# NERSC/swin_v2_weather

Hardware: AMD Instinct MI355X
Metric: ERA5 samples/sec (73x721x1440) swin_73var depth12 (higher is better)
Workload: dtype bf16

## Files before the change

### include/swv2.h

```cpp
#ifndef SWV2_H
#define SWV2_H
#include <stddef.h>
#include <stdint.h>

#ifdef __cplusplus
extern "C" {
#endif

#define SWV2_VERSION 113

enum {
    SWV2_OK = 0,
    SWV2_ERR_INVALID = -1,
    SWV2_ERR_UNSUPPORTED = -2,
    SWV2_ERR_LAUNCH = -3
};

int swv2_version(void);
const char* swv2_last_error(void);

int swv2_attn_geometry(int L, int head_dim, int* Lp, int* DP);

int swv2_attn_fwd_regime(int L, int head_dim, int has_bias, int dbg);

// ... 352 lines not shown
    const float* b2;
    const float* gamma;
    const float* beta;
    const float* scale;
    void* hpre;
    void* a2;
    float* mean;
    float* rstd;
    float* y;
    int M, C, hidden, rows_per_sample;
    float eps;
} swv2_mlp_args;
int swv2_mlp_supported(int C, int hidden);
int swv2_mlp_recompute_supported(int C, int hidden);
int swv2_mlp_fwd(const swv2_mlp_args* a, void* stream);

typedef struct {
    const float* dy;
    const void* a2;
    const float* mean;
    const float* rstd;
    const float* gamma;
    const float* scale;
    const void* hpre;
    const void* w2t;
    const void* w1t;
    void* da2;
    void* dh;
    float* dx;
    float* dgamma;
// ... 116 lines not shown
```

### swin_v2_weather_amd/_lib.py

```python
from __future__ import annotations

import ctypes as C
import os
import subprocess
import threading

HERE = os.path.dirname(os.path.abspath(__file__))
CSRC = os.path.join(HERE, "csrc")
LIB_PATH = os.environ.get("SWV2_LIB") or os.path.join(HERE, "libswv2.so")
SOURCES = ["capi.hip", "attn.hip", "attn2.hip", "attn_bwd_stream.hip", "attn_wide.hip", "attn_d256.hip", "gemm.hip", "gemm_rw.hip", "gemm_tn.hip", "gemm_tn_slab.hip", "rowops.hip", "lamb.hip", "block.hip", "cpb.hip", "mlp.hip", "proj_ln.hip", "dataio.hip", "packed.hip", "score.hip", "stats.hip", "quantile.hip", "ensemble.hip", "loss_l1.hip", "loss_l2.hip", "sht.hip", "regrid.hip", "events.hip", "fss.hip"]

ABI_VERSION = 113

_lib = None
_lock = threading.Lock()


class Swv2Error(RuntimeError):
    pass


def build_library(force: bool = False, verbose: bool = False) -> str:
    import glob
    srcs = [os.path.join(CSRC, s) for s in SOURCES]
# ... 257 lines not shown
    "swv2_era5_select_normalize": (_I, [_P, _P, _P, _P, _P] + [_I] * 10 + [_P]),
    "swv2_era5_zenith": (_I, [_P, _P, _I, _I, _I, _I, _I, _I, _P]),
    "swv2_era5_static": (_I, [_P, _P, _I, _I, _I, _I, _I, _I, _P]),
    "swv2_era5_select_normalize_i16": (_I, [_P] * 8 + [_I] * 10 + [_P]),
    "swv2_era5_unpack_i16": (_I, [_P, _P, _P, _P, _I, _I, _I, _P]),
    "swv2_era5_pack_i16": (_I, [_P, _P, _P, _P, _I, _I, _I, _P]),
    "swv2_pack_range_ws_bytes": (C.c_size_t, [_I, _I, _I]),
    "swv2_pack_range": (_I, [_P, _I, _I, _I, _I, _P, _P, _P, C.c_size_t, _P]),
    "swv2_proj_ln_supported": (_I, [_I, _I, _I]),
    "swv2_proj_ln_bwd_ws_floats": (C.c_size_t, [_I, _I]),
    "swv2_proj_ln_fwd": (_I, [C.POINTER(ProjLnArgs), _P]),
    "swv2_proj_ln_bwd": (_I, [C.POINTER(ProjLnBwdArgs), _P]),
    "swv2_mlp_supported": (_I, [_I, _I]),
    "swv2_mlp_recompute_supported": (_I, [_I, _I]),
    "swv2_mlp_fwd": (_I, [C.POINTER(MlpArgs), _P]),
    "swv2_mlp_bwd_ws_floats": (C.c_size_t, [_I, _I]),
    "swv2_mlp_bwd": (_I, [C.POINTER(MlpBwdArgs), _P]),
    "swv2_cpb_fwd": (_I, [_P, _P, _P, _P, _P, _P, _I, _I, _I, _I, _F, _P]),
    "swv2_cpb_bwd": (_I, [_P, _P, _P, _P, _P, _P, _P, _P, _P, _I, _I, _I, _I, _F, _P]),
    "swv2_cpb_bwd_ws": (_I, [_P, _P, _P, _P, _P, _P, _P, _P, _P, _I, _I, _I, _I, _F, _P, C.c_size_t, _P]),
    "swv2_cpb_bwd_ws_bytes": (C.c_size_t, [_I, _I, _I, _I]),
    "swv2_cpb_fwd_multi": (_I, [_P, _I, _P, _P, _I, _I, _I, _I, _F, _P]),
    "swv2_cpb_bwd_multi_ws_bytes": (C.c_size_t, [_I, _I, _I, _I, _I]),
    "swv2_cpb_bwd_multi": (_I, [_P, _I, _P, _I, _P, _P, _I, _I, _I, _I, _F, _P, C.c_size_t, _P]),
    "swv2_block_plan": (_I, [C.POINTER(BlockDesc), C.POINTER(BlockPlan)]),
    "swv2_block_step_id": (_I, [_I]),
    "swv2_block_step_name": (C.c_char_p, [_I]),
    "swv2_block_fwd": (_I, [C.POINTER(BlockDesc), _P]),
    "swv2_block_bwd": (_I, [C.POINTER(BlockDesc), _P]),
}
# ... 29 lines not shown
```

### swin_v2_weather_amd/csrc/gemm_common.h

```cpp
#pragma once
#include <cstdlib>
#include "common.h"

int swv2_tn_wide_launch(const swv2_operand* y, const swv2_operand* x, float* part, float* dbpart, int M, int N, int K, int S, hipStream_t st);

int swv2_rw_dx128_launch(const swv2_operand* a, const void* w, const swv2_epilogue* e, int M, hipStream_t st);

size_t swv2_tn_slab_ws_bytes(int C, int hidden, int heads_dp);
bool swv2_tn_slab_covers(const swv2_wgrad_item* it, size_t ws_bytes);
int swv2_tn_slab_launch(const swv2_wgrad_item* it, void* ws, size_t ws_bytes, const swv2_ln_partials* ln, hipStream_t st);

inline int swv2_env_switch(const char* name) { const char* v = getenv(name); return v ? atoi(v) : 1; }
inline int swv2_gemm_wide() { return swv2_env_switch("SWV2_GEMM_WIDE"); }
inline int swv2_wide_persist() { return swv2_env_switch("SWV2_WIDE_PERSIST"); }

namespace {

constexpr int BM = 128, BN = 128, BK = 64;
constexpr int KCH = BK / 8;
constexpr int NTHREADS = 256;

__device__ __forceinline__ int swz(int r, int kc) { return r * BK + ((kc ^ ((r >> 1) & 7)) << 3); }

__device__ __forceinline__ void erf_parts(float x, float& erf_v, float& gauss) {
    const float z = fabsf(x) * 0.70710678118654752f;
// ... 28 lines not shown
__device__ __forceinline__ uint16_t gelu_tab_arg(int i) { return (uint16_t)(((i / GT_HALF) << 15) | (GT_LO + i % GT_HALF)); }

template <int ESZ, bool SIGNED = true>
__device__ __forceinline__ uint32_t gelu_tab_off2(uint32_t w, bool& bad) {
    const u16x2_t a = __builtin_bit_cast(u16x2_t, w & 0x7fff7fffu);
    const u16x2_t lo = {(unsigned short)GT_LO, (unsigned short)GT_LO};
    const u16x2_t mx = {(unsigned short)(GT_HALF - 1), (unsigned short)(GT_HALF - 1)};
    const u16x2_t idx = a - lo;
    const u16x2_t idc = __builtin_elementwise_min(idx, mx);
    bad = bad || (__builtin_bit_cast(uint32_t, idx) != __builtin_bit_cast(uint32_t, idc));
    if constexpr (!SIGNED) return __builtin_bit_cast(uint32_t, (u16x2_t)(idc * (unsigned short)ESZ));
    const u16x2_t sg = __builtin_bit_cast(u16x2_t, w) >> 15;
    const u16x2_t half = {(unsigned short)GT_HALF, (unsigned short)GT_HALF};
    const u16x2_t off = (idc + sg * half) * (unsigned short)ESZ;
    return __builtin_bit_cast(uint32_t, off);
}

struct LoadDesc {
    const void* ptr;
    const int32_t* rowidx;
    const float* aux0;
    const float* aux1;
    const float* aux2;
    const float* aux3;
    long ld;
    int M, K;
    int p0, p1, p2, p3;
    uint32_t mg0, mg1, mg2;
};

// ... 258 lines not shown
```

### swin_v2_weather_amd/csrc/gemm_tn_slab.hip

```cpp
#include "gemm_common.h"
#pragma clang diagnostic ignored "-Wc++20-extensions"

namespace {

#ifdef SWV2_SLAB_PART_F32
typedef float sl_part_t;
#else
typedef uint16_t sl_part_t;
#endif
constexpr int SL_TH = 512;
constexpr int SL_SMEM = 160 * 1024;
constexpr int SL_IDX_CAP = 4096;
enum { F_ROW = 0, F_ROWG = 1, F_F32 = 2, F_F32G = 3, F_HEAD = 4 };

#ifdef SWV2_SLAB_STAMPS
#define SWV2_STAMPS
#endif
#include "stamps.h"

__device__ __forceinline__ uint4 sl_gelu8_tab(uint4 w, const unsigned char* tab0, bool& bad) {
    const uint32_t in[4] = {w.x, w.y, w.z, w.w};
    uint32_t out[4], off[4];
    u16x2_t mx = {0, 0};
    const u16x2_t lo = {(unsigned short)GT_LO, (unsigned short)GT_LO};
// ... 15 lines not shown

struct SlOp {
    const void* ptr;
    const int32_t* rowidx;
    int ld;
    int heads, parts, Lp, DP;
    uint32_t mgLp, mgDP, mgH;
};
struct SlProd {
    SlOp y, x;
    sl_part_t* part;
    float* dbpart;
    int M, N, K;
    int first, wgs, ntile;
};
struct SlArgs { SlProd p[4]; unsigned long long* stamps; };

template <int W>
__device__ __forceinline__ int sl_swz(int r, int u) {
    if constexpr ((W * 2) % 256 == 0) return u ^ (r & 7);
    else { static_assert((W * 2) % 128 == 0, "slab width"); return u ^ ((r >> 1) & 3); }
}

template <int FY, int FX, int TN, int TK, int WGN, int WGK, int SR, int NS, bool INPLACE = false>
__device__ __forceinline__ void slab_job(const SlProd& P, const int j, unsigned char* __restrict__ smem, [[maybe_unused]] unsigned long long* stamps) {
    static_assert(WGN * WGK == 8, "8 waves");
    constexpr int IA = TN / (16 * WGN), JB = TK / (16 * WGK);
    static_assert(IA * 16 * WGN == TN && JB * 16 * WGK == TK, "wave tiles");
    constexpr bool XF32 = FX == F_F32 || FX == F_F32G;
    constexpr int YP = TN * 2, XP = TK * 2;
    constexpr int YB = SR * TN * 2, XB = SR * TK * (XF32 ? 4 : 2), STG = YB + XB;
    constexpr int NY = YB / 1024, NX = XB / 1024, NTOT = NY + NX;
    static_assert(YB % 1024 == 0 && XB % 1024 == 0, "whole DMA instructions");
    constexpr int NIW = (NTOT + 7) / 8, NREM = NTOT % 8, D = NS - 1;
    constexpr int OFF_TAB = 0, TABB = FX == F_ROWG ? (GT_N * 2 + 1023) / 1024 * 1024 : 0;
    constexpr int OFF_IDX = OFF_TAB + TABB, IDXB = FX == F_F32G ? SL_IDX_CAP * 4 : 0;
    constexpr int OFF_SLOT = OFF_IDX + IDXB;
    constexpr int OFF_XB = OFF_SLOT + NS * STG, XBB = (XF32 && !INPLACE) ? SR * TK * 2 : 0;
    static_assert(OFF_XB + XBB <= SL_SMEM, "LDS budget");
    static_assert(!INPLACE || XF32, "in-place conversion: fp32 operands only");
    constexpr int KS = SR / 32;

    const int tid = threadIdx.x, lane = tid & 63, wave = __builtin_amdgcn_readfirstlane(tid >> 6);
    const int fr = lane & 15, g = lane >> 4;
    const int wgn = wave / WGK, wgk = wave - wgn * WGK;
    const int n_w = wgn * (TN / WGN), k_w = wgk * (TK / WGK);
    const int ntile = P.ntile, ntk = P.K / TK;
    const int slice = j / ntile, tile = j - slice * ntile, S = P.wgs / ntile;
    const int n0 = (tile / ntk) * TN, k0 = (tile % ntk) * TK;
    const int M = P.M, T = (M + SR - 1) / SR;
    const int nst = slice < T ? (T - slice + S - 1) / S : 0;
    auto stage_of = [&](int i) { return slice + i * S; };
    const uint32_t lds0 = (uint32_t)(uintptr_t)smem + OFF_SLOT;
    uint16_t* const xbs = (uint16_t*)(smem + OFF_XB);
    uint16_t* const tab = (uint16_t*)(smem + OFF_TAB);
    int32_t* const idxs = (int32_t*)(smem + OFF_IDX);

    if constexpr (FX == F_ROWG) {
        for (int i = tid; i < GT_N; i += SL_TH) tab[i] = f2bf(gelu_f(bf2f(gelu_tab_arg(i))));
    }
    constexpr int HS = SL_IDX_CAP / 2 / SR, RING = 2 * HS;
    auto fill_idx = [&](int h0) {
        for (int i = tid; i < HS * SR; i += SL_TH) {
            const int ti = h0 + i / SR;
            const int m = stage_of(ti) * SR + (i % SR);
            idxs[(ti % RING) * SR + (i % SR)] = (ti < nst && m < M) ? P.x.rowidx[m] : -1;
        }
    };
    if constexpr (FX == F_F32G) { fill_idx(0); fill_idx(HS); }
    if constexpr (FX == F_ROWG || FX == F_F32G) __syncthreads();

    int orow[NIW];
    uint32_t ocol[NIW];
#pragma unroll
    for (int q = 0; q < NIW; ++q) {
        const int ii = 8 * q + wave;
        if (ii < NY) {
            const int o = ii * 1024 + lane * 16;
            if constexpr (FY == F_ROW) {
                const int row = o / YP, rem = o - row * YP, pu = rem >> 5, u = sl_swz<TN>(row, pu);
                orow[q] = row; ocol[q] = (uint32_t)(n0 + u * 16 + ((rem >> 4) & 1) * 8);
            } else {
                static_assert(FY == F_HEAD, "dY kinds");
                const int blk = o / (SR * 32), rem = o - blk * (SR * 32), row = rem >> 5, col = n0 + blk * 16 + ((rem >> 4) & 1) * 8;
                const int ph = fdiv(col, P.y.DP, P.y.mgDP), jj = col - ph * P.y.DP, part = fdiv(ph, P.y.heads, P.y.mgH), hd = ph - part * P.y.heads;
// ... 75 lines not shown
    glf.tab = nullptr;

    auto tr_row = [&](const uint16_t* slab, auto wtag, int r0, int c) -> bf16x4 {
        constexpr int W = decltype(wtag)::value;
        const int row = r0 + 4 * g + (fr >> 2);
        return lds_tr_read(slab + row * W + (sl_swz<W>(row, c >> 4) << 4) + (fr & 3) * 4);
    };
    auto tr_head = [&](const uint16_t* slab, int r0, int c) -> bf16x4 {
        const int row = r0 + 4 * g + (fr >> 2);
        return lds_tr_read(slab + (c >> 4) * (SR * 16) + row * 16 + (fr & 3) * 4);
    };

    STAMP_DECL(8)
    STAMP_START();
    if (nst > 0) {
#pragma unroll
        for (int d = 0; d < D; ++d) issue(min(d, nst - 1), d);
        STAMP_DRAINED(7);
        for (int t = 0; t < nst; ++t) {
            if (NREM == 0 || wave < NREM) asm volatile("s_waitcnt vmcnt(%0)" : : "n"((D - 1) * NIW) : "memory");
            else asm volatile("s_waitcnt vmcnt(%0)" : : "n"((D - 1) * (NIW - 1)) : "memory");
            STAMP_DRAINED(0);
            __builtin_amdgcn_sched_barrier(0);
            __builtin_amdgcn_s_barrier();
            __builtin_amdgcn_sched_barrier(0);
            STAMP_DRAINED(1);
            const int ti_n = min(t + D, nst - 1), slot_n = (t + D) % NS;
            if constexpr (FX == F_F32G) {
                if (t > 0 && t % HS == 0 && t + HS < nst) fill_idx(t + HS);
            }
// ... 140 lines not shown
    }
#endif
    if (want_db && fr == 0) {
#pragma unroll
        for (int i = 0; i < IA; ++i)
            if (i % WGK == wgk) {
#pragma unroll
                for (int r = 0; r < 4; ++r) P.dbpart[(size_t)slice * P.N + n0 + n_w + 16 * i + 4 * g + r] = accdb[i / WGK][r];
            }
    }
}

__global__ __launch_bounds__(SL_TH) void gemm_tn_slab_c128_kernel(SlArgs a) {
    __shared__ __attribute__((aligned(1024))) unsigned char smem[SL_SMEM];
    const int b = blockIdx.x;
    if (b < a.p[1].first) slab_job<F_ROW, F_ROWG, 128, 512, 1, 8, 32, 3>(a.p[0], b - a.p[0].first, smem, a.stamps);
    else if (b < a.p[2].first) slab_job<F_ROW, F_F32, 512, 128, 8, 1, 32, 3>(a.p[1], b - a.p[1].first, smem, a.stamps);
    else if (b < a.p[3].first) slab_job<F_ROW, F_HEAD, 128, 128, 2, 4, 64, 4>(a.p[2], b - a.p[2].first, smem, a.stamps);
    else slab_job<F_HEAD, F_F32G, 384, 128, 8, 1, 32, 3>(a.p[3], b - a.p[3].first, smem, a.stamps);
}
__global__ __launch_bounds__(SL_TH) void gemm_tn_slab_c192_kernel(SlArgs a) {
    __shared__ __attribute__((aligned(1024))) unsigned char smem[SL_SMEM];
    const int b = blockIdx.x;
    if (b < a.p[1].first) slab_job<F_ROW, F_ROWG, 192, 384, 1, 8, 32, 3>(a.p[0], b - a.p[0].first, smem, a.stamps);
    else if (b < a.p[2].first) slab_job<F_ROW, F_F32, 384, 192, 8, 1, 32, 3>(a.p[1], b - a.p[1].first, smem, a.stamps);
    else if (b < a.p[3].first) slab_job<F_ROW, F_HEAD, 192, 256, 2, 4, 32, 4>(a.p[2], b - a.p[2].first, smem, a.stamps);
    else slab_job<F_HEAD, F_F32G, 384, 192, 8, 1, 32, 3, true>(a.p[3], b - a.p[3].first, smem, a.stamps);
}

struct SlLnRed { const float* ws[2]; float* dg[2]; float* db[2]; int n[2]; int C; };
struct SlRed { float* dW; float* db; const int32_t* nmap; const int32_t* kmap; const sl_part_t* part; const float* dbpart;
               int ldw, N, K, TN, TK, WGK, IA, JB, ntk, S, first, dbfirst; };
struct SlRedArgs { SlRed p[4]; int total, dbtotal; SlLnRed ln; int cpw; };
__global__ __launch_bounds__(512) void tn_slab_reduce_kernel(SlRedArgs a) {
    __shared__ f32x4 red[8][64];
    const int b = blockIdx.x;
    const int lane = threadIdx.x & 63, sg = threadIdx.x >> 6;
    if (b >= a.total + a.dbtotal) {
        const int bb = b - a.total - a.dbtotal, per_set = (2 * a.ln.C + 15) / 16;
        const int set = bb / per_set, col = threadIdx.x & 15, sl = threadIdx.x >> 4;
        const int jc = (bb - set * per_set) * 16 + col;
        float sum = 0.f;
// ... 227 lines not shown
        q.dbfirst = dbfirst;
        dbfirst += cdiv(p.N, 64);
    }
    r.total = rfirst;
    r.dbtotal = dbfirst;
    int lnblocks = 0;
    if (ln && ln->C > 0) {
        for (int i = 0; i < 2; ++i) { r.ln.ws[i] = ln->ws[i]; r.ln.dg[i] = ln->dgamma[i]; r.ln.db[i] = ln->dbeta[i]; r.ln.n[i] = ln->n[i]; }
        r.ln.C = ln->C;
        lnblocks = 2 * cdiv(2 * ln->C, 16);
    }
#ifdef SWV2_SLAB_STAMPS
    if (ws_bytes >= pl.total + (size_t)first * 64) a.stamps = (unsigned long long*)((char*)ws + ws_bytes - (size_t)first * 64);
    { static int once = 0; if (!once++) fprintf(stderr, "slab plan: workgroups %d %d %d %d\n", pl.wgs[0], pl.wgs[1], pl.wgs[2], pl.wgs[3]); }
#endif
    if (pl.set == 0) hipLaunchKernelGGL(gemm_tn_slab_c128_kernel, dim3(first), dim3(SL_TH), 0, st, a);
    else hipLaunchKernelGGL(gemm_tn_slab_c192_kernel, dim3(first), dim3(SL_TH), 0, st, a);
    hipLaunchKernelGGL(tn_slab_reduce_kernel, dim3(rfirst + dbfirst + lnblocks), dim3(512), 0, st, r);
    SWV2_CHECK_LAUNCH("swv2_block_wgrad(slab)");
    return 0;
}
```

### swin_v2_weather_amd/csrc/mlp.hip

```cpp
#include <cstdlib>
#include "gemm_common.h"
#include "ln_common.h"

namespace {

constexpr int MLP_MAX_HIDDEN = 2048;
constexpr int MLP_RECOMP_MAX_HIDDEN = 1024;

struct MlpFwd {
    const float* x; const uint16_t* w1; const float* b1; const uint16_t* w2; const float* b2;
    const float* gamma; const float* beta; const float* scale;
    uint16_t* hpre; uint16_t* a2; float* mean; float* rstd; float* y;
    int M, hidden, rows_per_sample; float eps;
};

template <int C, int MT>
__global__ __launch_bounds__(256, 2) void mlp_fwd_kernel(const MlpFwd a) {
    constexpr int KS = C / 32, NT = C / 16;
    constexpr int P1 = C + 8, P2 = 40;
    constexpr int W1E = 32 * P1, W2E = C * P2;
    constexpr int NCHUNK = 4 * C;
    constexpr int SPT = (NCHUNK + 255) / 256;
    constexpr int ROWS = 64 * MT;
    constexpr int PX = C + 8;
    constexpr int PA = C + 8;
    constexpr int EWAVE = 16 * PA * 2 + 16 * 2 * 4;
    constexpr int WBYTES = 2 * (W1E + W2E) * 2, XBYTES = ROWS * PX * 2, EBYTES = 4 * EWAVE;
    constexpr int SBYTES = WBYTES > XBYTES ? (WBYTES > EBYTES ? WBYTES : EBYTES) : (XBYTES > EBYTES ? XBYTES : EBYTES);
// ... 33 lines not shown
                *(u32x4*)(W1s + (idx / (C / 8)) * P1 + 8 * (idx % (C / 8))) = s1[i];
                const int q = idx & 3;
                uint16_t* row = W2s + (idx >> 2) * P2 + 4 * (q >> 1);
                *(u32x2*)(row + 16 * (q & 1)) = (u32x2){s2[i][0], s2[i][1]};
                *(u32x2*)(row + 16 * (q & 1) + 8) = (u32x2){s2[i][2], s2[i][3]};
            }
        }
    };
#ifdef SWV2_MLP_STAMPS
    unsigned long long tacc[8] = {0, 0, 0, 0, 0, 0, 0, 0}, tprev = __builtin_amdgcn_s_memtime();
#define STAMP(i) do { const unsigned long long t_ = __builtin_amdgcn_s_memtime(); tacc[i] += t_ - tprev; tprev = t_; } while (0)
#else
#define STAMP(i)
#endif
    issue(0);
    for (int i = tid; i < hid; i += 256) b1s[i] = a.b1[i];
    for (int i = tid; i < C; i += 256) { cs[i] = a.b2[i]; cs[C + i] = a.gamma[i]; cs[2 * C + i] = a.beta[i]; }
    for (int i = tid; i < GT_N; i += 256) gtab[i] = f2bf(gelu_f(bf2f(gelu_tab_arg(i))));

    {
        constexpr int UNITS = ROWS * (C / 4);
#pragma unroll
        for (int i = 0; i < UNITS / 256; ++i) {
            const int u = tid + 256 * i, row = u / (C / 4), c4 = u % (C / 4);
            const f32x4 v = *(const f32x4*)(a.x + (size_t)min(wg_row0 + row, a.M - 1) * C + 4 * c4);
            *(bf16x4*)(smem + row * PX + 4 * c4) = f2bf4(v);
        }
    }
    __syncthreads();
    bf16x8 xf[MT][KS];
#pragma unroll
    for (int mt = 0; mt < MT; ++mt)
#pragma unroll
        for (int ks = 0; ks < KS; ++ks)
            xf[mt][ks] = *(const bf16x8*)(smem + (wave * 16 * MT + 16 * mt + fr) * PX + 32 * ks + 8 * g);
    __syncthreads();

    f32x4 yacc[MT][NT];
#pragma unroll
    for (int mt = 0; mt < MT; ++mt)
#pragma unroll
        for (int t = 0; t < NT; ++t) yacc[mt][t] = (f32x4){0.f, 0.f, 0.f, 0.f};

// ... 165 lines not shown
#endif
}

template <int C, int MT>
void launch_mlp_fwd(const MlpFwd& k, hipStream_t st) {
    hipLaunchKernelGGL((mlp_fwd_kernel<C, MT>), dim3(cdiv(k.M, 64 * MT)), dim3(256), 0, st, k);
}

struct MlpBwd {
    const float* dy; const uint16_t* a2; const float* mean; const float* rstd; const float* gamma; const float* scale;
    const uint16_t* hpre; const uint16_t* w2t; const uint16_t* w1t;
    uint16_t* da2; uint16_t* dh; float* dx; float* ws;
    int M, hidden, rows_per_sample;
    float* zero; long zero_n;
    const float* x; const uint16_t* w1; const float* b1;
};

template <int C, int MT, bool RECOMP>
__global__ __launch_bounds__(256, (C >= 192 && MT == 2) ? 1 : 2) void mlp_bwd_kernel(const MlpBwd a) {
    if (a.zero) {
        for (long i = ((long)blockIdx.x * 256 + threadIdx.x) * 4; i < a.zero_n; i += (long)gridDim.x * 256 * 4)
            *(f32x4*)(a.zero + i) = (f32x4){0.f, 0.f, 0.f, 0.f};
    }
    constexpr int KS = C / 32, NT = C / 16;
    constexpr int P1 = C + 8, P2 = 40;
    constexpr int W1E = 32 * P1, W2E = C * P2;
    constexpr int NCHUNK = 4 * C;
    constexpr int SPT = (NCHUNK + 255) / 256;
    constexpr int PY = C + 4;
    constexpr int ROWS = 64 * MT, PX = C + 8;
    constexpr int XBYTES = ROWS * PX * 2;
    constexpr int GBYTES = LnBwdShape<C, 256, ROWS>::RPP * 2 * C * 4;
    constexpr int B1BYTES = RECOMP ? MLP_RECOMP_MAX_HIDDEN * 4 : 0;
    constexpr int WBYTES = 2 * (W1E + W2E) * 2, EBYTES = 4 * 16 * PY * 4, PBYTES = XBYTES + GBYTES, WB1 = WBYTES + B1BYTES;
    constexpr int SBYTES0 = WB1 > EBYTES ? (WB1 > PBYTES ? WB1 : PBYTES) : (EBYTES > PBYTES ? EBYTES : PBYTES);
    constexpr int SBYTES = (SBYTES0 + 15) / 16 * 16;
    __shared__ __attribute__((aligned(16))) unsigned char smem_raw[SBYTES];
    uint16_t* smem = (uint16_t*)smem_raw;
// ... 1 lines not shown
    typedef uint32_t u32x4 __attribute__((ext_vector_type(4)));
    typedef uint32_t u32x2 __attribute__((ext_vector_type(2)));

    const int tid = threadIdx.x, lane = tid & 63, wave = tid >> 6, fr = lane & 15, g = lane >> 4;
    const int wg_row0 = blockIdx.x * ROWS;
    const int row0 = wg_row0 + wave * (16 * MT);
    const int hid = a.hidden, nch = hid / 32;
    constexpr int PHS = 72;
    __shared__ __attribute__((aligned(16))) uint16_t hst_all[4 * 16 * MT * PHS];
    uint16_t* const Hst = hst_all + wave * (16 * MT * PHS);
    constexpr int LBASE = SBYTES + 4 * 16 * MT * PHS * 2;
    constexpr bool ONE_WG = C >= 192 && MT == 2;
    constexpr bool GTAB = LBASE + GT_N * 4 <= (ONE_WG ? 156 : 80) * 1024;
    constexpr bool GHALF = !GTAB && !ONE_WG && (LBASE + GT_HALF * 4 <= 80 * 1024);
    __shared__ __attribute__((aligned(16))) float ggtab[GTAB ? GT_N : (GHALF ? GT_HALF : 4)];
    if (GTAB)
        for (int i = tid; i < GT_N; i += 256) ggtab[i] = gelu_grad_f(bf2f(gelu_tab_arg(i)));
    else if (GHALF)
        for (int i = tid; i < GT_HALF; i += 256) ggtab[i] = gelu_grad_f(bf2f(gelu_tab_arg(i)));

    static_assert(32 * P1 <= W2E, "the row-major fc1 chunk of the recompute mode fits the W1^T chunk's slot");
    u32x4 s1[SPT], s2[SPT];
    auto issue = [&](int ch) {
#pragma unroll
        for (int i = 0; i < SPT; ++i) {
            const int idx = min(tid + 256 * i, NCHUNK - 1);
            s1[i] = *(const u32x4*)(a.w2t + (size_t)(32 * ch + idx / (C / 8)) * C + 8 * (idx % (C / 8)));
            if constexpr (RECOMP) s2[i] = *(const u32x4*)(a.w1 + (size_t)(32 * ch + idx / (C / 8)) * C + 8 * (idx % (C / 8)));
            else s2[i] = *(const u32x4*)(a.w1t + (size_t)(idx >> 2) * hid + 32 * ch + 8 * (idx & 3));
        }
    };
    auto commit = [&](int buf) {
        uint16_t* W1s = smem + buf * (W1E + W2E);
        uint16_t* W2s = W1s + W1E;
// ... 25 lines not shown
    };
    auto commit_hq = [&]() {
        if constexpr (!RECOMP)
#pragma unroll
        for (int p_ = 0; p_ < 2 * MT; ++p_) {
            const int u = lane + 64 * p_, row = u >> 3, c8 = u & 7;
            *(u32x4*)(Hst + row * PHS + 8 * c8) = hq[p_];
        }
    };
    bf16x8 xf1[RECOMP ? MT : 1][KS];
#ifdef SWV2_MLP_STAMPS
    unsigned long long tacc[8] = {0, 0, 0, 0, 0, 0, 0, 0}, tprev = __builtin_amdgcn_s_memtime();
#endif
    issue(0);
    issue_hq(0);
    if constexpr (RECOMP) {
        constexpr int UNITS = ROWS * (C / 4);
#pragma unroll
        for (int i = 0; i < UNITS / 256; ++i) {
            const int u = tid + 256 * i, row = u / (C / 4), c4 = u % (C / 4);
            const f32x4 v = *(const f32x4*)(a.x + (size_t)min(wg_row0 + row, a.M - 1) * C + 4 * c4);
            *(bf16x4*)(smem + row * PX + 4 * c4) = f2bf4(v);
        }
        __syncthreads();
#pragma unroll
        for (int mt = 0; mt < MT; ++mt)
#pragma unroll
            for (int ks = 0; ks < KS; ++ks)
                xf1[mt][ks] = *(const bf16x8*)(smem + (wave * 16 * MT + 16 * mt + fr) * PX + 32 * ks + 8 * g);
        __syncthreads();
// ... 10 lines not shown
        f32x4 dgm = {0.f, 0.f, 0.f, 0.f}, dbt = {0.f, 0.f, 0.f, 0.f};
#pragma unroll 1
        for (int pb = 0; pb < NPASS; pb += BATCH) {
            f32x4 d4[BATCH];
            u32x2 a4[BATCH];
            float mu[BATCH], rs[BATCH], sc[BATCH];
#pragma unroll
            for (int i = 0; i < BATCH; ++i) {
                const int rc = min(wg_row0 + (pb + i) * RPP + rg, a.M - 1);
                d4[i] = *(const f32x4*)(a.dy + (size_t)rc * C + c0);
                a4[i] = *(const u32x2*)(a.a2 + (size_t)rc * C + c0);
                mu[i] = a.mean[rc];
                rs[i] = a.rstd[rc];
                sc[i] = a.scale ? a.scale[rc / a.rows_per_sample] : 1.f;
            }
#pragma unroll
            for (int i = 0; i < BATCH; ++i) {
                const int row = (pb + i) * RPP + rg;
                const float once = (act && wg_row0 + row < a.M) ? 1.f : 0.f;
                const float av[4] = {__uint_as_float(a4[i][0] << 16), __uint_as_float(a4[i][0] & 0xffff0000u),
                                     __uint_as_float(a4[i][1] << 16), __uint_as_float(a4[i][1] & 0xffff0000u)};
                float gg[4], xh[4], t1 = 0.f, t2 = 0.f;
#pragma unroll
                for (int e = 0; e < 4; ++e) {
                    const float d = act ? sc[i] * d4[i][e] : 0.f;
                    xh[e] = (av[e] - mu[i]) * rs[i];
                    gg[e] = d * gm[e];
                    dgm[e] = fmaf(once * d, xh[e], dgm[e]);
                    dbt[e] = fmaf(once, d, dbt[e]);
                    t1 += gg[e];
// ... 176 lines not shown
#pragma unroll
    for (int mt = 0; mt < MT; ++mt) {
        if constexpr (!DY_ALL) load_dy(mt);
#pragma unroll
        for (int t = 0; t < NT; ++t) *(f32x4*)(Ys + fr * PY + 16 * t + 4 * g) = yacc[mt][t];
        __syncthreads();
        const int rbase = row0 + 16 * mt;
#pragma unroll
        for (int p = 0; p < EPASS; ++p) {
            const int u = lane + 64 * p, row = u / (C / 4), c4 = u % (C / 4);
            const size_t off = (size_t)min(rbase + row, a.M - 1) * C + 4 * c4;
            *(f32x4*)(a.dx + off) = dyv[DY_ALL ? mt : 0][p] + *(const f32x4*)(Ys + row * PY + 4 * c4);
        }
        if (mt + 1 < MT) __syncthreads();
    }
#ifdef SWV2_MLP_STAMPS
    STAMP(7);
    if (lane == 0 && (blockIdx.x % 97) == 0) {
        unsigned long long* o = (unsigned long long*)(a.ws + (size_t)gridDim.x * 2 * C) + ((blockIdx.x / 97) * 4 + wave) * 8;
        for (int i = 0; i < 8; ++i) o[i] = tacc[i];
    }
#endif
}

template <int C, int MT>
void launch_mlp_bwd(const MlpBwd& k, hipStream_t st) {
    if (k.hpre) hipLaunchKernelGGL((mlp_bwd_kernel<C, MT, false>), dim3(cdiv(k.M, 64 * MT)), dim3(256), 0, st, k);
    else hipLaunchKernelGGL((mlp_bwd_kernel<C, MT, true>), dim3(cdiv(k.M, 64 * MT)), dim3(256), 0, st, k);
}

}

extern "C" int swv2_mlp_supported(int C, int hidden) {
    return (C == 32 || C == 64 || C == 96 || C == 128 || C == 192 || C == 256) && hidden > 0 && hidden % 32 == 0 && hidden <= MLP_MAX_HIDDEN;
}

extern "C" int swv2_mlp_recompute_supported(int C, int hidden) {
    return swv2_mlp_supported(C, hidden) && hidden <= MLP_RECOMP_MAX_HIDDEN;
}

extern "C" int swv2_mlp_fwd(const swv2_mlp_args* a, void* stream) {
    SWV2_CHECK_ARG(a && a->x && a->w1 && a->b1 && a->w2 && a->b2 && a->gamma && a->beta && a->a2 && a->mean &&
                       a->rstd && a->y, "swv2_mlp_fwd: null pointer");
    SWV2_CHECK_ARG(a->M > 0 && a->rows_per_sample > 0, "swv2_mlp_fwd: M and rows_per_sample must be positive");
    if (!swv2_mlp_supported(a->C, a->hidden)) {
        swv2_set_error("swv2_mlp_fwd: C=%d hidden=%d not instantiated (C in {32,64,96,128,192,256}, hidden %% 32 == 0); "
                       "use swv2_linear + swv2_ln_residual_fwd", a->C, a->hidden);
        return SWV2_ERR_UNSUPPORTED;
    }
    MlpFwd k = {a->x, (const uint16_t*)a->w1, a->b1, (const uint16_t*)a->w2, a->b2, a->gamma, a->beta, a->scale,
                (uint16_t*)a->hpre, (uint16_t*)a->a2, a->mean, a->rstd, a->y, a->M, a->hidden, a->rows_per_sample, a->eps};
    hipStream_t st = (hipStream_t)stream;
    const bool mt2 = a->M >= 128 * 256;
    switch (a->C) {
        case 32: mt2 ? launch_mlp_fwd<32, 2>(k, st) : launch_mlp_fwd<32, 1>(k, st); break;
        case 64: mt2 ? launch_mlp_fwd<64, 2>(k, st) : launch_mlp_fwd<64, 1>(k, st); break;
        case 96: mt2 ? launch_mlp_fwd<96, 2>(k, st) : launch_mlp_fwd<96, 1>(k, st); break;
        case 128: mt2 ? launch_mlp_fwd<128, 2>(k, st) : launch_mlp_fwd<128, 1>(k, st); break;
        case 192: {
            a->hidden > 1024 ? launch_mlp_fwd<192, 2>(k, st) : launch_mlp_fwd<192, 1>(k, st);
            break;
        }
        case 256: launch_mlp_fwd<256, 1>(k, st); break;
    }
    SWV2_CHECK_LAUNCH("swv2_mlp_fwd");
    return SWV2_OK;
}
// ... 4 lines not shown

int swv2_mlp_bwd_impl(const swv2_mlp_bwd_args* a, void* stream, int* deferred, float* zero, long zero_n) {
    SWV2_CHECK_ARG(!zero || (zero_n % 4 == 0 && ((uintptr_t)zero & 15) == 0), "swv2_mlp_bwd: the zeroed buffer must be 16-byte aligned / sized");
    SWV2_CHECK_ARG(a && a->dy && a->a2 && a->mean && a->rstd && a->gamma && a->w2t && a->da2 && a->dh &&
                       a->dx && a->dgamma && a->dbeta && a->ws, "swv2_mlp_bwd: null pointer");
    SWV2_CHECK_ARG((a->hpre && a->w1t) || (a->x && a->w1 && a->b1),
                   "swv2_mlp_bwd: either the saved pre-activation (hpre, w1t) or the recompute inputs (x, w1, b1) are needed");
    SWV2_CHECK_ARG(a->hpre || swv2_mlp_recompute_supported(a->C, a->hidden), "swv2_mlp_bwd: recompute mode needs hidden <= %d", MLP_RECOMP_MAX_HIDDEN);
    SWV2_CHECK_ARG(a->M > 0 && a->rows_per_sample > 0, "swv2_mlp_bwd: M and rows_per_sample must be positive");
    if (!swv2_mlp_supported(a->C, a->hidden)) {
        swv2_set_error("swv2_mlp_bwd: C=%d hidden=%d not instantiated; use swv2_ln_residual_bwd + swv2_linear", a->C, a->hidden);
        return SWV2_ERR_UNSUPPORTED;
    }
    MlpBwd k = {a->dy, (const uint16_t*)a->a2, a->mean, a->rstd, a->gamma, a->scale, (const uint16_t*)a->hpre,
                (const uint16_t*)a->w2t, (const uint16_t*)a->w1t, (uint16_t*)a->da2, (uint16_t*)a->dh, a->dx, a->ws, a->M,
                a->hidden, a->rows_per_sample, zero, zero_n, a->x, (const uint16_t*)a->w1, a->b1};
    hipStream_t st = (hipStream_t)stream;
    const bool mt2 = a->M >= 128 * 256;
    switch (a->C) {
        case 32: mt2 ? launch_mlp_bwd<32, 2>(k, st) : launch_mlp_bwd<32, 1>(k, st); break;
        case 64: mt2 ? launch_mlp_bwd<64, 2>(k, st) : launch_mlp_bwd<64, 1>(k, st); break;
        case 96: mt2 ? launch_mlp_bwd<96, 2>(k, st) : launch_mlp_bwd<96, 1>(k, st); break;
        case 128: mt2 ? launch_mlp_bwd<128, 2>(k, st) : launch_mlp_bwd<128, 1>(k, st); break;
        case 192: {
            launch_mlp_bwd<192, 1>(k, st);
            break;
        }
        case 256: launch_mlp_bwd<256, 1>(k, st); break;
    }
    const bool two = (a->C <= 128) && mt2;
    if (deferred) *deferred = cdiv(a->M, two ? 128 : 64);
    else swv2_launch_ln_partials_reduce(a->ws, a->dgamma, a->dbeta, cdiv(a->M, two ? 128 : 64), a->C, st);
// ... 4 lines not shown
```

Baseline: 227.3.

## Precompute GELU lookup tables once in global memory and DMA them into LDS

Replaces the per-workgroup computation of the GELU and GELU-gradient lookup tables (in the MLP forward/backward kernels and the slab weight-gradient kernel) with a one-time fill kernel that writes device-global tables. Each workgroup now copies the table into LDS with async DMA loads overlapped with its other prologue loads. The backward kernel's buffer zeroing is moved from the start of the kernel to the end. The change adds a per-device init state machine with events, stream-capture handling and a mutex, which adds host-side bookkeeping and a waitcnt before first table use.

```diff
diff --git a/include/swv2.h b/include/swv2.h
--- a/include/swv2.h
+++ b/include/swv2.h
@@ -390,6 +390,8 @@
 int swv2_mlp_supported(int C, int hidden);
 int swv2_mlp_recompute_supported(int C, int hidden);
 int swv2_mlp_fwd(const swv2_mlp_args* a, void* stream);
+
+int swv2_gelu_tables_copy(void* gelu_bf16, void* grad_f32, void* stream);
 
 typedef struct {
     const float* dy;
diff --git a/swin_v2_weather_amd/_lib.py b/swin_v2_weather_amd/_lib.py
--- a/swin_v2_weather_amd/_lib.py
+++ b/swin_v2_weather_amd/_lib.py
@@ -295,6 +295,7 @@
     "swv2_mlp_supported": (_I, [_I, _I]),
     "swv2_mlp_recompute_supported": (_I, [_I, _I]),
     "swv2_mlp_fwd": (_I, [C.POINTER(MlpArgs), _P]),
+    "swv2_gelu_tables_copy": (_I, [_P, _P, _P]),
     "swv2_mlp_bwd_ws_floats": (C.c_size_t, [_I, _I]),
     "swv2_mlp_bwd": (_I, [C.POINTER(MlpBwdArgs), _P]),
     "swv2_cpb_fwd": (_I, [_P, _P, _P, _P, _P, _P, _I, _I, _I, _I, _F, _P]),
diff --git a/swin_v2_weather_amd/csrc/gemm_common.h b/swin_v2_weather_amd/csrc/gemm_common.h
--- a/swin_v2_weather_amd/csrc/gemm_common.h
+++ b/swin_v2_weather_amd/csrc/gemm_common.h
@@ -9,6 +9,9 @@
 size_t swv2_tn_slab_ws_bytes(int C, int hidden, int heads_dp);
 bool swv2_tn_slab_covers(const swv2_wgrad_item* it, size_t ws_bytes);
 int swv2_tn_slab_launch(const swv2_wgrad_item* it, void* ws, size_t ws_bytes, const swv2_ln_partials* ln, hipStream_t st);
+
+struct swv2_gelu_tables_t { const uint16_t* gelu; const float* grad; };
+int swv2_gelu_tables_get(hipStream_t st, swv2_gelu_tables_t* out);
 
 inline int swv2_env_switch(const char* name) { const char* v = getenv(name); return v ? atoi(v) : 1; }
 inline int swv2_gemm_wide() { return swv2_env_switch("SWV2_GEMM_WIDE"); }
@@ -67,6 +70,17 @@
     const u16x2_t half = {(unsigned short)GT_HALF, (unsigned short)GT_HALF};
     const u16x2_t off = (idc + sg * half) * (unsigned short)ESZ;
     return __builtin_bit_cast(uint32_t, off);
+}
+
+template <int BYTES, int NW>
+__device__ __forceinline__ void gelu_tab_dma(const void* tab, uint32_t lds_addr, int wave, int lane) {
+    static_assert(BYTES % 1024 == 0, "whole DMA instructions");
+#pragma unroll
+    for (int q = 0; q < (BYTES / 1024 + NW - 1) / NW; ++q) {
+        const int ii = wave + NW * q;
+        if (NW * (q + 1) <= BYTES / 1024 || ii < BYTES / 1024)
+            dma_x4(tab, (uint32_t)(ii * 1024 + lane * 16), lds_addr + (uint32_t)(ii * 1024));
+    }
 }
 
 struct LoadDesc {
diff --git a/swin_v2_weather_amd/csrc/gemm_tn_slab.hip b/swin_v2_weather_amd/csrc/gemm_tn_slab.hip
--- a/swin_v2_weather_amd/csrc/gemm_tn_slab.hip
+++ b/swin_v2_weather_amd/csrc/gemm_tn_slab.hip
@@ -53,7 +53,7 @@
     int M, N, K;
     int first, wgs, ntile;
 };
-struct SlArgs { SlProd p[4]; unsigned long long* stamps; };
+struct SlArgs { SlProd p[4]; unsigned long long* stamps; const uint16_t* gtab; };
 
 template <int W>
 __device__ __forceinline__ int sl_swz(int r, int u) {
@@ -62,7 +62,8 @@
 }
 
 template <int FY, int FX, int TN, int TK, int WGN, int WGK, int SR, int NS, bool INPLACE = false>
-__device__ __forceinline__ void slab_job(const SlProd& P, const int j, unsigned char* __restrict__ smem, [[maybe_unused]] unsigned long long* stamps) {
+__device__ __forceinline__ void slab_job(const SlProd& P, const int j, unsigned char* __restrict__ smem, [[maybe_unused]] unsigned long long* stamps,
+                                         [[maybe_unused]] const uint16_t* gtab) {
     static_assert(WGN * WGK == 8, "8 waves");
     constexpr int IA = TN / (16 * WGN), JB = TK / (16 * WGK);
     static_assert(IA * 16 * WGN == TN && JB * 16 * WGK == TK, "wave tiles");
@@ -92,12 +93,8 @@
     auto stage_of = [&](int i) { return slice + i * S; };
     const uint32_t lds0 = (uint32_t)(uintptr_t)smem + OFF_SLOT;
     uint16_t* const xbs = (uint16_t*)(smem + OFF_XB);
-    uint16_t* const tab = (uint16_t*)(smem + OFF_TAB);
     int32_t* const idxs = (int32_t*)(smem + OFF_IDX);
 
-    if constexpr (FX == F_ROWG) {
-        for (int i = tid; i < GT_N; i += SL_TH) tab[i] = f2bf(gelu_f(bf2f(gelu_tab_arg(i))));
-    }
     constexpr int HS = SL_IDX_CAP / 2 / SR, RING = 2 * HS;
     auto fill_idx = [&](int h0) {
         for (int i = tid; i < HS * SR; i += SL_TH) {
@@ -107,7 +104,7 @@
         }
     };
     if constexpr (FX == F_F32G) { fill_idx(0); fill_idx(HS); }
-    if constexpr (FX == F_ROWG || FX == F_F32G) __syncthreads();
+    if constexpr (FX == F_F32G) __syncthreads();
 
     int orow[NIW];
     uint32_t ocol[NIW];
@@ -213,6 +210,7 @@
     STAMP_DECL(8)
     STAMP_START();
     if (nst > 0) {
+        if constexpr (FX == F_ROWG) gelu_tab_dma<GT_N * 2, 8>(gtab, (uint32_t)(uintptr_t)smem + OFF_TAB, wave, lane);
 #pragma unroll
         for (int d = 0; d < D; ++d) issue(min(d, nst - 1), d);
         STAMP_DRAINED(7);
@@ -383,18 +381,18 @@
 __global__ __launch_bounds__(SL_TH) void gemm_tn_slab_c128_kernel(SlArgs a) {
     __shared__ __attribute__((aligned(1024))) unsigned char smem[SL_SMEM];
     const int b = blockIdx.x;
-    if (b < a.p[1].first) slab_job<F_ROW, F_ROWG, 128, 512, 1, 8, 32, 3>(a.p[0], b - a.p[0].first, smem, a.stamps);
-    else if (b < a.p[2].first) slab_job<F_ROW, F_F32, 512, 128, 8, 1, 32, 3>(a.p[1], b - a.p[1].first, smem, a.stamps);
-    else if (b < a.p[3].first) slab_job<F_ROW, F_HEAD, 128, 128, 2, 4, 64, 4>(a.p[2], b - a.p[2].first, smem, a.stamps);
-    else slab_job<F_HEAD, F_F32G, 384, 128, 8, 1, 32, 3>(a.p[3], b - a.p[3].first, smem, a.stamps);
+    if (b < a.p[1].first) slab_job<F_ROW, F_ROWG, 128, 512, 1, 8, 32, 3>(a.p[0], b - a.p[0].first, smem, a.stamps, a.gtab);
+    else if (b < a.p[2].first) slab_job<F_ROW, F_F32, 512, 128, 8, 1, 32, 3>(a.p[1], b - a.p[1].first, smem, a.stamps, a.gtab);
+    else if (b < a.p[3].first) slab_job<F_ROW, F_HEAD, 128, 128, 2, 4, 64, 4>(a.p[2], b - a.p[2].first, smem, a.stamps, a.gtab);
+    else slab_job<F_HEAD, F_F32G, 384, 128, 8, 1, 32, 3>(a.p[3], b - a.p[3].first, smem, a.stamps, a.gtab);
 }
 __global__ __launch_bounds__(SL_TH) void gemm_tn_slab_c192_kernel(SlArgs a) {
     __shared__ __attribute__((aligned(1024))) unsigned char smem[SL_SMEM];
     const int b = blockIdx.x;
-    if (b < a.p[1].first) slab_job<F_ROW, F_ROWG, 192, 384, 1, 8, 32, 3>(a.p[0], b - a.p[0].first, smem, a.stamps);
-    else if (b < a.p[2].first) slab_job<F_ROW, F_F32, 384, 192, 8, 1, 32, 3>(a.p[1], b - a.p[1].first, smem, a.stamps);
-    else if (b < a.p[3].first) slab_job<F_ROW, F_HEAD, 192, 256, 2, 4, 32, 4>(a.p[2], b - a.p[2].first, smem, a.stamps);
-    else slab_job<F_HEAD, F_F32G, 384, 192, 8, 1, 32, 3, true>(a.p[3], b - a.p[3].first, smem, a.stamps);
+    if (b < a.p[1].first) slab_job<F_ROW, F_ROWG, 192, 384, 1, 8, 32, 3>(a.p[0], b - a.p[0].first, smem, a.stamps, a.gtab);
+    else if (b < a.p[2].first) slab_job<F_ROW, F_F32, 384, 192, 8, 1, 32, 3>(a.p[1], b - a.p[1].first, smem, a.stamps, a.gtab);
+    else if (b < a.p[3].first) slab_job<F_ROW, F_HEAD, 192, 256, 2, 4, 32, 4>(a.p[2], b - a.p[2].first, smem, a.stamps, a.gtab);
+    else slab_job<F_HEAD, F_F32G, 384, 192, 8, 1, 32, 3, true>(a.p[3], b - a.p[3].first, smem, a.stamps, a.gtab);
 }
 
 struct SlLnRed { const float* ws[2]; float* dg[2]; float* db[2]; int n[2]; int C; };
@@ -652,6 +650,9 @@
     if (ws_bytes >= pl.total + (size_t)first * 64) a.stamps = (unsigned long long*)((char*)ws + ws_bytes - (size_t)first * 64);
     { static int once = 0; if (!once++) fprintf(stderr, "slab plan: workgroups %d %d %d %d\n", pl.wgs[0], pl.wgs[1], pl.wgs[2], pl.wgs[3]); }
 #endif
+    swv2_gelu_tables_t gt;
+    if (const int rc = swv2_gelu_tables_get(st, &gt)) return rc;
+    a.gtab = gt.gelu;
     if (pl.set == 0) hipLaunchKernelGGL(gemm_tn_slab_c128_kernel, dim3(first), dim3(SL_TH), 0, st, a);
     else hipLaunchKernelGGL(gemm_tn_slab_c192_kernel, dim3(first), dim3(SL_TH), 0, st, a);
     hipLaunchKernelGGL(tn_slab_reduce_kernel, dim3(rfirst + dbfirst + lnblocks), dim3(512), 0, st, r);
diff --git a/swin_v2_weather_amd/csrc/mlp.hip b/swin_v2_weather_amd/csrc/mlp.hip
--- a/swin_v2_weather_amd/csrc/mlp.hip
+++ b/swin_v2_weather_amd/csrc/mlp.hip
@@ -1,4 +1,6 @@
+#include <atomic>
 #include <cstdlib>
+#include <mutex>
 #include "gemm_common.h"
 #include "ln_common.h"
 
@@ -12,6 +14,7 @@
     const float* gamma; const float* beta; const float* scale;
     uint16_t* hpre; uint16_t* a2; float* mean; float* rstd; float* y;
     int M, hidden, rows_per_sample; float eps;
+    const uint16_t* gtab;
 };
 
 template <int C, int MT>
@@ -75,9 +78,9 @@
 #define STAMP(i)
 #endif
     issue(0);
+    gelu_tab_dma<GT_N * 2, 4>(a.gtab, (uint32_t)(uintptr_t)gtab, __builtin_amdgcn_readfirstlane(wave), lane);
     for (int i = tid; i < hid; i += 256) b1s[i] = a.b1[i];
     for (int i = tid; i < C; i += 256) { cs[i] = a.b2[i]; cs[C + i] = a.gamma[i]; cs[2 * C + i] = a.beta[i]; }
-    for (int i = tid; i < GT_N; i += 256) gtab[i] = f2bf(gelu_f(bf2f(gelu_tab_arg(i))));
 
     {
         constexpr int UNITS = ROWS * (C / 4);
@@ -88,6 +91,7 @@
             *(bf16x4*)(smem + row * PX + 4 * c4) = f2bf4(v);
         }
     }
+    asm volatile("s_waitcnt vmcnt(0)" ::: "memory");
     __syncthreads();
     bf16x8 xf[MT][KS];
 #pragma unroll
@@ -283,14 +287,11 @@
     int M, hidden, rows_per_sample;
     float* zero; long zero_n;
     const float* x; const uint16_t* w1; const float* b1;
+    const float* ggtab;
 };
 
 template <int C, int MT, bool RECOMP>
 __global__ __launch_bounds__(256, (C >= 192 && MT == 2) ? 1 : 2) void mlp_bwd_kernel(const MlpBwd a) {
-    if (a.zero) {
-        for (long i = ((long)blockIdx.x * 256 + threadIdx.x) * 4; i < a.zero_n; i += (long)gridDim.x * 256 * 4)
-            *(f32x4*)(a.zero + i) = (f32x4){0.f, 0.f, 0.f, 0.f};
-    }
     constexpr int KS = C / 32, NT = C / 16;
     constexpr int P1 = C + 8, P2 = 40;
     constexpr int W1E = 32 * P1, W2E = C * P2;
@@ -322,10 +323,6 @@
     constexpr bool GTAB = LBASE + GT_N * 4 <= (ONE_WG ? 156 : 80) * 1024;
     constexpr bool GHALF = !GTAB && !ONE_WG && (LBASE + GT_HALF * 4 <= 80 * 1024);
     __shared__ __attribute__((aligned(16))) float ggtab[GTAB ? GT_N : (GHALF ? GT_HALF : 4)];
-    if (GTAB)
-        for (int i = tid; i < GT_N; i += 256) ggtab[i] = gelu_grad_f(bf2f(gelu_tab_arg(i)));
-    else if (GHALF)
-        for (int i = tid; i < GT_HALF; i += 256) ggtab[i] = gelu_grad_f(bf2f(gelu_tab_arg(i)));
 
     static_assert(32 * P1 <= W2E, "the row-major fc1 chunk of the recompute mode fits the W1^T chunk's slot");
     u32x4 s1[SPT], s2[SPT];
@@ -381,6 +378,8 @@
 #endif
     issue(0);
     issue_hq(0);
+    if constexpr (GTAB) gelu_tab_dma<GT_N * 4, 4>(a.ggtab, (uint32_t)(uintptr_t)ggtab, __builtin_amdgcn_readfirstlane(wave), lane);
+    else if constexpr (GHALF) gelu_tab_dma<GT_HALF * 4, 4>(a.ggtab, (uint32_t)(uintptr_t)ggtab, __builtin_amdgcn_readfirstlane(wave), lane);
     if constexpr (RECOMP) {
         constexpr int UNITS = ROWS * (C / 4);
 #pragma unroll
@@ -421,6 +420,7 @@
                 rs[i] = a.rstd[rc];
                 sc[i] = a.scale ? a.scale[rc / a.rows_per_sample] : 1.f;
             }
+            if ((GTAB || GHALF) && pb == 0) asm volatile("s_waitcnt vmcnt(0)" ::: "memory");
 #pragma unroll
             for (int i = 0; i < BATCH; ++i) {
                 const int row = (pb + i) * RPP + rg;
@@ -627,6 +627,10 @@
         }
         if (mt + 1 < MT) __syncthreads();
     }
+    if (a.zero) {
+        for (long i = ((long)blockIdx.x * 256 + threadIdx.x) * 4; i < a.zero_n; i += (long)gridDim.x * 256 * 4)
+            *(f32x4*)(a.zero + i) = (f32x4){0.f, 0.f, 0.f, 0.f};
+    }
 #ifdef SWV2_MLP_STAMPS
     STAMP(7);
     if (lane == 0 && (blockIdx.x % 97) == 0) {
@@ -642,6 +646,83 @@
     else hipLaunchKernelGGL((mlp_bwd_kernel<C, MT, true>), dim3(cdiv(k.M, 64 * MT)), dim3(256), 0, st, k);
 }
 
+__device__ __attribute__((aligned(1024))) uint16_t gelu_tab_dev[GT_N];
+__device__ __attribute__((aligned(1024))) float gelu_grad_tab_dev[GT_N];
+
+__global__ __launch_bounds__(256) void gelu_tables_fill_kernel() {
+    const int i = blockIdx.x * 256 + threadIdx.x;
+    if (i < GT_N) {
+        const float x = bf2f(gelu_tab_arg(i));
+        gelu_tab_dev[i] = f2bf(gelu_f(x));
+        gelu_grad_tab_dev[i] = gelu_grad_f(x);
+    }
+}
+
+constexpr int GT_MAX_DEV = 64;
+struct GeluTabDev {
+    std::atomic<int> state{0};
+    swv2_gelu_tables_t t{nullptr, nullptr};
+    hipEvent_t ev = nullptr;
+    bool recorded = false;
+};
+GeluTabDev gelu_tab_devs[GT_MAX_DEV];
+std::mutex gelu_tab_mu;
+
+}
+
+int swv2_gelu_tables_get(hipStream_t st, swv2_gelu_tables_t* out) {
+    int dev = 0;
+    if (hipGetDevice(&dev) != hipSuccess || dev < 0 || dev >= GT_MAX_DEV) {
+        swv2_set_error("swv2: GELU tables: no current device below %d", GT_MAX_DEV);
+        return SWV2_ERR_LAUNCH;
+    }
+    GeluTabDev& d = gelu_tab_devs[dev];
+    if (d.state.load(std::memory_order_acquire) == 2) { *out = d.t; return SWV2_OK; }
+    std::lock_guard<std::mutex> lock(gelu_tab_mu);
+    if (d.state.load(std::memory_order_relaxed) == 0) {
+        void *pg = nullptr, *pd = nullptr;
+        if (hipGetSymbolAddress(&pg, HIP_SYMBOL(gelu_tab_dev)) != hipSuccess || hipGetSymbolAddress(&pd, HIP_SYMBOL(gelu_grad_tab_dev)) != hipSuccess ||
+            hipEventCreateWithFlags(&d.ev, hipEventDisableTiming) != hipSuccess) {
+            (void)hipGetLastError();
+            swv2_set_error("swv2: GELU tables: no device address / event on device %d", dev);
+            return SWV2_ERR_LAUNCH;
+        }
+        d.t = {(const uint16_t*)pg, (const float*)pd};
+        d.state.store(1, std::memory_order_release);
+    }
+    hipStreamCaptureStatus cap = hipStreamCaptureStatusNone;
+    if (hipStreamIsCapturing(st, &cap) != hipSuccess) { (void)hipGetLastError(); cap = hipStreamCaptureStatusNone; }
+    if (cap == hipStreamCaptureStatusNone && d.state.load(std::memory_order_relaxed) == 1 && d.recorded) {
+        if (hipEventQuery(d.ev) == hipSuccess) {
+            d.state.store(2, std::memory_order_release);
+            *out = d.t;
+            return SWV2_OK;
+        }
+        (void)hipGetLastError();
+    }
+    if (d.state.load(std::memory_order_relaxed) != 2) {
+        hipLaunchKernelGGL(gelu_tables_fill_kernel, dim3(cdiv(GT_N, 256)), dim3(256), 0, st);
+        if (cap == hipStreamCaptureStatusNone) d.recorded = hipEventRecord(d.ev, st) == hipSuccess;
+        SWV2_CHECK_LAUNCH("swv2: GELU tables");
+    }
+    *out = d.t;
+    return SWV2_OK;
+}
+
+extern "C" int swv2_gelu_tables_copy(void* gelu_bf16, void* grad_f32, void* stream) {
+    SWV2_CHECK_ARG(gelu_bf16 || grad_f32, "swv2_gelu_tables_copy: null pointers");
+    hipStream_t st = (hipStream_t)stream;
+    swv2_gelu_tables_t gt;
+    if (const int rc = swv2_gelu_tables_get(st, &gt)) return rc;
+    hipError_t e = hipSuccess;
+    if (gelu_bf16) e = hipMemcpyAsync(gelu_bf16, gt.gelu, GT_N * sizeof(uint16_t), hipMemcpyDeviceToDevice, st);
+    if (e == hipSuccess && grad_f32) e = hipMemcpyAsync(grad_f32, gt.grad, GT_N * sizeof(float), hipMemcpyDeviceToDevice, st);
+    if (e != hipSuccess) {
+        (void)hipGetLastError();
+        swv2_set_error("swv2_gelu_tables_copy: copy failed: %s", hipGetErrorString(e));
+        return SWV2_ERR_LAUNCH;
+    }
+    return SWV2_OK;
 }
 
 extern "C" int swv2_mlp_supported(int C, int hidden) {
@@ -661,9 +742,11 @@
                        "use swv2_linear + swv2_ln_residual_fwd", a->C, a->hidden);
         return SWV2_ERR_UNSUPPORTED;
     }
+    hipStream_t st = (hipStream_t)stream;
+    swv2_gelu_tables_t gt;
+    if (const int rc = swv2_gelu_tables_get(st, &gt)) return rc;
     MlpFwd k = {a->x, (const uint16_t*)a->w1, a->b1, (const uint16_t*)a->w2, a->b2, a->gamma, a->beta, a->scale,
-                (uint16_t*)a->hpre, (uint16_t*)a->a2, a->mean, a->rstd, a->y, a->M, a->hidden, a->rows_per_sample, a->eps};
-    hipStream_t st = (hipStream_t)stream;
+                (uint16_t*)a->hpre, (uint16_t*)a->a2, a->mean, a->rstd, a->y, a->M, a->hidden, a->rows_per_sample, a->eps, gt.gelu};
     const bool mt2 = a->M >= 128 * 256;
     switch (a->C) {
         case 32: mt2 ? launch_mlp_fwd<32, 2>(k, st) : launch_mlp_fwd<32, 1>(k, st); break;
@@ -698,8 +781,11 @@
     }
     MlpBwd k = {a->dy, (const uint16_t*)a->a2, a->mean, a->rstd, a->gamma, a->scale, (const uint16_t*)a->hpre,
                 (const uint16_t*)a->w2t, (const uint16_t*)a->w1t, (uint16_t*)a->da2, (uint16_t*)a->dh, a->dx, a->ws, a->M,
-                a->hidden, a->rows_per_sample, zero, zero_n, a->x, (const uint16_t*)a->w1, a->b1};
+                a->hidden, a->rows_per_sample, zero, zero_n, a->x, (const uint16_t*)a->w1, a->b1, nullptr};
     hipStream_t st = (hipStream_t)stream;
+    swv2_gelu_tables_t gt;
+    if (const int rc = swv2_gelu_tables_get(st, &gt)) return rc;
+    k.ggtab = gt.grad;
     const bool mt2 = a->M >= 128 * 256;
     switch (a->C) {
         case 32: mt2 ? launch_mlp_bwd<32, 2>(k, st) : launch_mlp_bwd<32, 1>(k, st); break;
```

After: 227.1. Within noise of the previous version (-0.1%).
